# jamie8johnson/cqs

Hardware: AMD Instinct MI355X
Metric: queries/sec @k=20 (brute-force cosine scan + top-k, 768-d fp32) (higher is better)
Workload: dtype f32; 1 GPU; BASELINE configs[1]: 1000000 x 768 fp32 unit vectors, 1 query per step, brute-force cosine top-20; mode=single, rows_per_gpu=1000000, total_rows=1000000, dim=768, k=20, parallelism=single GPU, ranks_seen=1

## Files before the change

cqs_amd/csrc/index_shadow.hip:

```cpp
#include <cstdlib>
#include <cstring>
#include <new>

#include "abi_guard.h"
#include "index_internal.h"
#include "scan_bf16.h"
#include "scan_i8.h"

namespace cqs_idx {

constexpr uint64_t kShadowAutoBytes = 1ull << 30;
constexpr uint64_t kShadowFreeMinBytes = 4ull << 30;
constexpr double kShadowFreeFrac = 0.10;
constexpr uint32_t kStatWords = 10, kStatCounts = 3, kStatI8 = 5, kStatI8Counts = 8;

struct Shadow {
    uint16_t* d_bf16 = nullptr;
    uint64_t cap = 0;
    int8_t* d_i8 = nullptr;
    float* d_i8_scale = nullptr;
    double r8 = 0.0, norm8 = 0.0;
    double r = 0.0;
    double norm = 0.0;
    unsigned long long* d_stats = nullptr;
    uint64_t* d_akeys = nullptr;
    uint32_t* d_acounts = nullptr;
    uint64_t* d_ekeys = nullptr;
    uint32_t* d_cert = nullptr;
    float* d_bq = nullptr;
    uint32_t* h_cert = nullptr;
    uint32_t* h_cert_dev = nullptr;
};

static void shadow_device_counts(cqs_hip_index* x, uint32_t first, uint64_t* certified, uint64_t* fallbacks) {
    unsigned long long c[2];
    if (!x->shadow || !x->shadow->d_stats || quiesce(x) != hipSuccess) return;
    hipError_t e = hipMemcpyAsync(c, x->shadow->d_stats + first, sizeof c, hipMemcpyDeviceToHost, x->stream);
    if (e == hipSuccess) e = hipStreamSynchronize(x->stream);
    if (e != hipSuccess) { (void)hipGetLastError(); return; }
    *certified += c[0];
    *fallbacks += c[1];
}

static void i8_free(Shadow* s) {
    hipFree(s->d_i8); hipFree(s->d_i8_scale);
    s->d_i8 = nullptr; s->d_i8_scale = nullptr;
}

void shadow_free(cqs_hip_index* x) {
    Shadow* s = x->shadow;
    if (!s) return;
    uint64_t c = 0, f = 0;
    shadow_device_counts(x, kStatCounts, &c, &f);
    x->stat_certified.fetch_add(c, std::memory_order_relaxed);
    x->stat_fallbacks.fetch_add(f, std::memory_order_relaxed);
    c = f = 0;
    shadow_device_counts(x, kStatI8Counts, &c, &f);
    x->stat_i8_certified.fetch_add(c, std::memory_order_relaxed);
    x->stat_i8_fallbacks.fetch_add(f, std::memory_order_relaxed);
    i8_free(s);
    hipFree(s->d_bf16); hipFree(s->d_stats); hipFree(s->d_akeys); hipFree(s->d_acounts); hipFree(s->d_ekeys);
    hipFree(s->d_cert); hipFree(s->d_bq); hipHostFree(s->h_cert);
    delete s;
    x->shadow = nullptr;
}

static int32_t shadow_convert(cqs_hip_index* x, uint64_t row0, bool* outlier) {
    Shadow* s = x->shadow;
    HIP_TRY(x, hipMemsetAsync(s->d_stats + 2, 0, sizeof(unsigned long long), x->stream));
    HIP_TRY(x, cqs::launch_shadow_build(x->d_rows, s->d_bf16, row0, x->n - row0, x->dim, cqs::shadow_gamma(x->dim),
                                        s->d_stats, x->stream));
    unsigned long long st[3];
    HIP_TRY(x, hipMemcpyAsync(st, s->d_stats, sizeof st, hipMemcpyDeviceToHost, x->stream));
    HIP_TRY(x, hipStreamSynchronize(x->stream));
    double r, m;
    memcpy(&r, &st[0], sizeof r);
    memcpy(&m, &st[1], sizeof m);
    s->r = r * (1.0 + 0x1p-30);
    s->norm = m * (1.0 + 0x1p-30);
    *outlier = st[2] != 0;
    return CQS_HIP_OK;
}

static int32_t i8_convert(cqs_hip_index* x, uint64_t row0) {
    Shadow* s = x->shadow;
    HIP_TRY(x, cqs::launch_i8_build(x->d_rows, s->d_i8, s->d_i8_scale, row0, x->n - row0, x->dim, cqs::i8_gamma(x->dim),
                                    s->d_stats + kStatI8, x->stream));
    unsigned long long st[2];
    HIP_TRY(x, hipMemcpyAsync(st, s->d_stats + kStatI8, sizeof st, hipMemcpyDeviceToHost, x->stream));
    HIP_TRY(x, hipStreamSynchronize(x->stream));
    double r, m;
    memcpy(&r, &st[0], sizeof r);
    memcpy(&m, &st[1], sizeof m);
    s->r8 = r * (1.0 + 0x1p-30);
    s->norm8 = m * (1.0 + 0x1p-30);
// ... 57 lines not shown
    int32_t rc = shadow_convert(x, n_old, &outlier);
    if (rc == CQS_HIP_OK && s->d_i8 && !outlier) rc = i8_convert(x, n_old);
    if (rc != CQS_HIP_OK) return rc;
    if (outlier) {
        shadow_free(x);
        x->last_error = "extend: a new row has a component of magnitude >= 2^64; bf16 shadow turned off";
    }
    return CQS_HIP_OK;
}

static bool dim_ok(uint32_t dim) { return dim % 8u == 0u && dim <= cqs::kShadowMaxDim; }
static const char* const kDimRule = ": dim must be a multiple of 8 and <= 2048";

static int32_t shadow_enable(cqs_hip_index* x, const char* what) {
    std::string pre(what);
    if (!dim_ok(x->dim)) return fail(x, CQS_HIP_ERR_INVALID, (pre + kDimRule).c_str());
    if (x->shadow) return CQS_HIP_OK;
    auto oom = [&](hipError_t e) { (void)hipGetLastError(); shadow_free(x); return fail(x, CQS_HIP_ERR_NOMEM, (pre + ": allocation").c_str(), e); };
    Shadow* s = x->shadow = new (std::nothrow) Shadow();
    if (!s) return oom(hipErrorOutOfMemory);
    const uint64_t cap = x->cap_rows ? x->cap_rows : 1;
    hipError_t e;
    if ((e = hipMalloc(&s->d_bf16, (size_t)cap * x->dim * sizeof(uint16_t))) != hipSuccess) return oom(e);
    s->cap = cap;
    unsigned long long* stats = nullptr;
    if ((e = hipMalloc(&stats, kStatWords * sizeof(unsigned long long))) != hipSuccess) return oom(e);
    if ((e = hipMemsetAsync(stats, 0, kStatWords * sizeof(unsigned long long), x->stream)) != hipSuccess) { hipFree(stats); return oom(e); }
    s->d_stats = stats;
    if ((e = hipMalloc(&s->d_akeys, (size_t)cqs::kShadowMaxQ * cqs::kMaxK * sizeof(uint64_t))) != hipSuccess) return oom(e);
    if ((e = hipMalloc(&s->d_acounts, (size_t)cqs::kShadowMaxQ * sizeof(uint32_t))) != hipSuccess) return oom(e);
    if ((e = hipMalloc(&s->d_ekeys, (size_t)cqs::kShadowMaxQ * (cqs::kMaxK - 1) * sizeof(uint64_t))) != hipSuccess) return oom(e);
    if ((e = hipMalloc(&s->d_cert, (size_t)cqs::kShadowMaxQ * sizeof(uint32_t))) != hipSuccess) return oom(e);
    if ((e = hipMalloc(&s->d_bq, (size_t)cqs::kShadowMaxQ * sizeof(float))) != hipSuccess) return oom(e);
    if ((e = hipHostMalloc(&s->h_cert, (size_t)cqs::kShadowMaxQ * sizeof(uint32_t), hipHostMallocDefault)) != hipSuccess) return oom(e);
    if (hipHostGetDevicePointer((void**)&s->h_cert_dev, s->h_cert, 0) != hipSuccess) {
        (void)hipGetLastError();
        s->h_cert_dev = nullptr;
    }
    bool outlier = false;
    const int32_t rc = shadow_convert(x, 0, &outlier);
    if (rc != CQS_HIP_OK) { shadow_free(x); return rc; }
    if (outlier) {
        shadow_free(x);
        return fail(x, CQS_HIP_ERR_INVALID, (pre + ": a finite row has a component of magnitude >= 2^64").c_str());
    }
    return CQS_HIP_OK;
}

static bool i8_dim_ok(uint32_t dim) { return cqs::i8_dim_ok(dim); }
static const char* const kI8DimRule = ": dim must be a multiple of 16 and <= 2048";
static int32_t i8_auto(cqs_hip_index* x) {
    Shadow* s = x->shadow;
    if (!s || s->d_i8) return CQS_HIP_OK;
    const char* env = getenv("CQS_HIP_SCAN_I8");
    if (env && env[0] == '0') return CQS_HIP_OK;
    if (!(env && env[0] == '1') && x->n * x->dim * sizeof(float) < kShadowAutoBytes) return CQS_HIP_OK;
    const std::string pre("int8 copy of the shadow not built (the bf16 copy serves every block)");
    if (!i8_dim_ok(x->dim)) { x->last_error = pre + kI8DimRule; return CQS_HIP_OK; }
    size_t free_b = 0, total_b = 0;
    if (hipMemGetInfo(&free_b, &total_b) != hipSuccess) {
        (void)hipGetLastError();
        x->last_error = pre + ": hipMemGetInfo failed";
        return CQS_HIP_OK;
    }
    const uint64_t need = i8_bytes(s->cap, x->dim);
    const uint64_t frac = (uint64_t)(kShadowFreeFrac * (double)total_b);
// ... 25 lines not shown
        (void)hipGetLastError();
        x->last_error = "bf16 shadow not built: hipMemGetInfo failed";
        return CQS_HIP_OK;
    }
    const uint64_t cap = x->cap_rows ? x->cap_rows : 1;
    const uint64_t need = cap * x->dim * sizeof(uint16_t) + (2ull * cqs::kMaxK + 2ull) * cqs::kShadowMaxQ * sizeof(uint64_t);
    const uint64_t frac = (uint64_t)(kShadowFreeFrac * (double)total_b);
    const uint64_t reserve = frac > kShadowFreeMinBytes ? frac : kShadowFreeMinBytes;
    if (free_b < need || free_b - need < reserve) {
        x->last_error = "bf16 shadow not built: the device would keep less than max(4 GiB, 10 %) of its memory free";
        return CQS_HIP_OK;
    }
    int32_t rc = shadow_enable(x, "bf16 shadow not built");
    if (rc == CQS_HIP_OK) rc = i8_auto(x);
    return rc == CQS_HIP_ERR_DEVICE ? rc : CQS_HIP_OK;
}

bool shadow_takes(const cqs_hip_index* x, uint32_t b, uint32_t k, bool gemv_only) {
    return x->shadow && b <= cqs::kShadowMaxQ && (gemv_only || !cqs::use_mfma(b, x->dim)) && cqs::shadow_kprime(k) >= k;
}

bool shadow_uses_i8(const cqs_hip_index* x, uint32_t b, uint32_t k) {
    return x->shadow && x->shadow->d_i8 && b <= cqs::kI8MaxQ && cqs::i8_k_ok(k);
}

int32_t shadow_pass(cqs_hip_index* x, const float* d_q, uint32_t nb, uint32_t k, const uint32_t* d_keep, uint32_t mode,
                    float threshold, uint64_t* out_keys, uint32_t* out_counts, hipStream_t st, const uint32_t** device_gate) {
    const Shadow* s = x->shadow;
    uint32_t* const cert = device_gate || !s->h_cert_dev ? s->d_cert : s->h_cert_dev;
    if (device_gate) *device_gate = cert;
    if (device_gate) HIP_TRY(x, order_after_last(x, st));
    const bool i8 = shadow_uses_i8(x, nb, k);
    const uint32_t kp = i8 ? cqs::i8_kprime(k) : cqs::shadow_kprime(k);
    if (i8) HIP_TRY(x, cqs::launch_i8_bound(d_q, nb, x->dim, s->r8, s->norm8, s->d_bq, st));
    else HIP_TRY(x, cqs::launch_shadow_bound(d_q, nb, x->dim, s->r, s->norm, s->d_bq, st));
    const cqs::ScanArgs a = scan_args(x, d_q, nb, kp + 1u, d_keep, mode, threshold, i8 ? sizeof(int8_t) : sizeof(uint16_t), true, nullptr, nullptr);
    const ShadowRows rows{i8 ? nullptr : s->d_bf16, i8 ? s->d_i8 : nullptr, s->d_i8_scale, s->d_bq};
    const int32_t rc = scan_select(x, a, st, &rows, s->d_akeys, s->d_acounts);
    if (rc == CQS_HIP_OK)
        HIP_TRY(x, cqs::launch_rescore_certify(x->d_rows, x->dim, d_q, nb, k, kp, mode, threshold, (uint32_t)x->row_base,
                                               s->d_bq, s->d_akeys, s->d_acounts, s->d_ekeys, out_keys, out_counts, cert,
                                               device_gate ? s->d_stats + kStatCounts : nullptr,
                                               device_gate && i8 ? s->d_stats + kStatI8Counts : nullptr, st));
    return rc;
}

hipError_t shadow_verdicts(cqs_hip_index* x, uint32_t nb, const uint32_t** h_cert) {
    const Shadow* s = x->shadow;
    *h_cert = s->h_cert;
    return s->h_cert_dev ? hipSuccess : hipMemcpyAsync(s->h_cert, s->d_cert, (size_t)nb * sizeof(uint32_t), hipMemcpyDeviceToHost, x->stream);
}

}

using namespace cqs_idx;

extern "C" {

int32_t cqs_hip_index_set_bf16_scan(cqs_hip_index* x, int32_t enable) CQS_ABI_TRY {
    if (!x || x->sh) return CQS_HIP_ERR_INVALID;
    std::lock_guard<std::mutex> g(x->mu);
    if (x->poisoned.load(std::memory_order_acquire)) return CQS_HIP_ERR_POISONED;
    HIP_TRY(x, hipSetDevice(x->device));
    HIP_TRY(x, quiesce(x));
    if (!enable) { shadow_free(x); return CQS_HIP_OK; }
    if (x->borrow) return fail(x, CQS_HIP_ERR_INVALID, "set_bf16_scan: index borrows its rows (they may change under the bound)");
    const int32_t rc = shadow_enable(x, "set_bf16_scan");
    return rc == CQS_HIP_OK ? i8_auto(x) : rc;
} CQS_ABI_CATCH(x)

void cqs_hip_index_bf16_stats(const cqs_hip_index* x, uint64_t* bytes, uint64_t* certified, uint64_t* fallbacks) CQS_ABI_TRY {
    uint64_t by = 0, c = 0, f = 0;
    if (x && !x->sh) {
        cqs_hip_index* m = const_cast<cqs_hip_index*>(x);
// ... 41 lines not shown
    for (uint32_t i = 0; i < b; ++i) {
        const float* q = queries + (size_t)i * x->dim;
        double s2 = 0.0;
        for (uint32_t d = 0; d < x->dim; ++d) s2 += (double)q[d] * (double)q[d];
        out_host[i] = cqs::shadow_query_bound(s2, s->r, s->norm, x->dim);
    }
    return CQS_HIP_OK;
} CQS_ABI_CATCH(x)

int32_t cqs_hip_debug_shadow_bound_i8(cqs_hip_index* x, const float* queries, uint32_t b, float* out_device, float* out_host) CQS_ABI_TRY {
    if (!x || x->sh || !queries || !out_device || !out_host || b == 0) return CQS_HIP_ERR_INVALID;
    std::lock_guard<std::mutex> g(x->mu);
    const Shadow* s = x->shadow;
    if (!s || !s->d_i8 || b > cqs::kShadowMaxQ) return CQS_HIP_ERR_INVALID;
    HIP_TRY(x, hipSetDevice(x->device));
    HIP_TRY(x, quiesce(x));
    float* d_q = nullptr;
    HIP_TRY(x, hipMalloc(&d_q, (size_t)b * x->dim * sizeof(float)));
    hipError_t e = hipMemcpyAsync(d_q, queries, (size_t)b * x->dim * sizeof(float), hipMemcpyHostToDevice, x->stream);
    if (e == hipSuccess) e = cqs::launch_i8_bound(d_q, b, x->dim, s->r8, s->norm8, s->d_bq, x->stream);
    if (e == hipSuccess) e = hipMemcpyAsync(out_device, s->d_bq, (size_t)b * sizeof(float), hipMemcpyDeviceToHost, x->stream);
    if (e == hipSuccess) e = hipStreamSynchronize(x->stream);
    hipFree(d_q);
    HIP_TRY(x, e);
    for (uint32_t i = 0; i < b; ++i) {
        const float* q = queries + (size_t)i * x->dim;
        double s2 = 0.0;
        for (uint32_t d = 0; d < x->dim; ++d) s2 += (double)q[d] * (double)q[d];
        out_host[i] = cqs::i8_query_bound(s2, s->r8, s->norm8, x->dim);
    }
    return CQS_HIP_OK;
} CQS_ABI_CATCH(x)

int32_t cqs_hip_debug_shadow_stats(cqs_hip_index* x, double* out) CQS_ABI_TRY {
    if (!x || x->sh || !out) return CQS_HIP_ERR_INVALID;
    std::lock_guard<std::mutex> g(x->mu);
    const Shadow* s = x->shadow;
    if (!s) return CQS_HIP_ERR_INVALID;
    out[0] = s->r; out[1] = s->norm;
    out[2] = s->d_i8 ? s->r8 : 0.0; out[3] = s->d_i8 ? s->norm8 : 0.0;
    return CQS_HIP_OK;
} CQS_ABI_CATCH(x)

int32_t cqs_hip_debug_shadow_rows(cqs_hip_index* x, uint32_t copy, uint64_t row0, uint64_t rows, void* out, float* out_scales) CQS_ABI_TRY {
    if (!x || x->sh || !out || (copy != 1u && copy != 2u) || (copy == 2u && !out_scales)) return CQS_HIP_ERR_INVALID;
    std::lock_guard<std::mutex> g(x->mu);
    const Shadow* s = x->shadow;
    if (!s || (copy == 2u && !s->d_i8) || row0 > x->n || rows > x->n - row0) return CQS_HIP_ERR_INVALID;
    if (rows == 0) return CQS_HIP_OK;
    HIP_TRY(x, hipSetDevice(x->device));
    HIP_TRY(x, quiesce(x));
    if (copy == 1u) {
        HIP_TRY(x, hipMemcpyAsync(out, s->d_bf16 + row0 * x->dim, (size_t)rows * x->dim * sizeof(uint16_t), hipMemcpyDeviceToHost, x->stream));
    } else {
        HIP_TRY(x, hipMemcpyAsync(out, s->d_i8 + row0 * x->dim, (size_t)rows * x->dim, hipMemcpyDeviceToHost, x->stream));
        HIP_TRY(x, hipMemcpyAsync(out_scales, s->d_i8_scale + row0, (size_t)rows * sizeof(float), hipMemcpyDeviceToHost, x->stream));
    }
    HIP_TRY(x, hipStreamSynchronize(x->stream));
    return CQS_HIP_OK;
} CQS_ABI_CATCH(x)

int32_t cqs_hip_debug_shadow_scores(cqs_hip_index* x, uint32_t copy, const float* queries, uint32_t b, uint32_t k,
                                    const uint32_t* keep_bitset, uint32_t mode, float threshold, float* out_scores,
                                    float* out_bq) CQS_ABI_TRY {
    if (!x || x->sh || !queries || !out_scores || !out_bq || b == 0 || copy > 2u || mode > CQS_HIP_MODE_PIPELINE) return CQS_HIP_ERR_INVALID;
    if (k == 0 || k > cqs::kMaxK) return CQS_HIP_ERR_INVALID;
// ... 39 lines not shown
```

cqs_amd/csrc/scan_bf16.h:

```cpp
#pragma once
#include <math.h>
#include <stdint.h>

#if defined(__HIPCC__)
#include <hip/hip_runtime.h>
#include "scan_kernels.h"
#define CQS_HD __host__ __device__
#else
#define CQS_HD
#endif

namespace cqs {

constexpr uint32_t kShadowMaxQ = 32;
constexpr uint32_t kShadowMaxDim = 2048;
constexpr uint32_t kShadowKMax = 1024;

inline uint32_t shadow_kprime(uint32_t k) {
    const uint32_t kp = 2u * k + 32u;
    return kp < kShadowKMax - 1u ? kp : kShadowKMax - 1u;
}

CQS_HD inline double shadow_gamma(uint32_t dim) {
    const double du = (double)dim * 0x1p-24;
    return du / (1.0 - du);
}

CQS_HD inline float round_up_f32(double v) {
    float f = (float)v;
    if ((double)f < v) f = nextafterf(f, INFINITY);
    return f;
}

CQS_HD inline float shadow_query_bound(double q_norm2, double r_max, double norm_max, uint32_t dim) {
    const double qn = sqrt(q_norm2) * (1.0 + 0x1p-40);
    if (!(qn * norm_max * (1.0 + shadow_gamma(dim)) < 0x1p100)) return INFINITY;
    return round_up_f32(qn * r_max * (1.0 + 0x1p-40) + (double)dim * 0x1p-140);
}

#if defined(__HIPCC__)
hipError_t launch_shadow_build(const float* rows, uint16_t* shadow, uint64_t row0, uint64_t n_rows, uint32_t dim,
                               double gamma, unsigned long long* stats, hipStream_t st);

hipError_t launch_shadow_bound(const float* q, uint32_t b, uint32_t dim, double r_max, double norm_max, float* bq,
                               hipStream_t st);

hipError_t launch_scan_bf16(const ScanArgs& a, const uint16_t* shadow, const float* bq, hipStream_t st);

hipError_t launch_rescore_certify(const float* rows, uint32_t dim, const float* q, uint32_t b, uint32_t k, uint32_t kprime,
                                  uint32_t mode, float thr, uint32_t row_base, const float* bq, const uint64_t* akeys,
                                  const uint32_t* acounts, uint64_t* ekeys, uint64_t* out_keys, uint32_t* out_counts,
                                  uint32_t* cert, unsigned long long* counters, unsigned long long* counters2, hipStream_t st);
#endif

}
```

cqs_amd/csrc/scan_bf16.hip:

```cpp
#include "scan_bf16.h"
#include "launch_util.h"
#include "rank_sort.h"
#include "scan_device.h"

namespace cqs {

static_assert(kShadowKMax == kMaxK, "shadow k' policy and the select agree on max k");

typedef float f4 __attribute__((ext_vector_type(4)));
typedef float f2 __attribute__((ext_vector_type(2)));
typedef unsigned u4 __attribute__((ext_vector_type(4)));
typedef __bf16 bf2 __attribute__((ext_vector_type(2)));

__device__ __forceinline__ float bf_lo(uint32_t w) { return __uint_as_float(w << 16); }
__device__ __forceinline__ float bf_hi(uint32_t w) { return __uint_as_float(w & 0xFFFF0000u); }
__device__ __forceinline__ float key_score(uint64_t key) {
    const uint32_t ok = (uint32_t)(key >> 32);
    return __uint_as_float((ok & 0x80000000u) ? (ok ^ 0x80000000u) : ~ok);
}

__global__ __launch_bounds__(256) void shadow_build_kernel(const float* __restrict__ rows, uint16_t* __restrict__ shadow,
                                                           uint64_t row0, uint64_t n_rows, uint32_t dim, double gamma,
                                                           unsigned long long* __restrict__ stats) {
    const int lane = threadIdx.x & 63;
    const uint64_t waves = (uint64_t)gridDim.x * (blockDim.x >> 6);
    for (uint64_t r = (uint64_t)blockIdx.x * (blockDim.x >> 6) + (threadIdx.x >> 6); r < n_rows; r += waves) {
        const float* xp = rows + (row0 + r) * dim;
        uint16_t* op = shadow + (row0 + r) * dim;
        double d2 = 0.0, n2 = 0.0, t2 = 0.0;
        bool fin = true, big = false;
        for (uint32_t i = (uint32_t)lane * 2u; i < dim; i += 128u) {
            const f2 v = *(const f2*)(xp + i);
            const bf2 h = __builtin_convertvector(v, bf2);
// ... 7 lines not shown
            n2 += (double)v.x * (double)v.x + (double)v.y * (double)v.y;
            t2 += (double)t0 * (double)t0 + (double)t1 * (double)t1;
        }
#pragma unroll
        for (int m = 32; m >= 1; m >>= 1) {
            d2 += __shfl_xor(d2, m, 64);
            n2 += __shfl_xor(n2, m, 64);
            t2 += __shfl_xor(t2, m, 64);
        }
        const bool all_fin = __ballot(!fin) == 0ull;
        const bool any_big = __ballot(big) != 0ull;
        if (lane == 0 && all_fin) {
            const double nx = sqrt(n2), nt = sqrt(t2);
            const double rb = sqrt(d2) + gamma * (nx + nt);
            atomicMax(&stats[0], (unsigned long long)__double_as_longlong(rb));
            atomicMax(&stats[1], (unsigned long long)__double_as_longlong(nx > nt ? nx : nt));
            if (any_big) atomicMax(&stats[2], 1ull);
        }
    }
}

hipError_t launch_shadow_build(const float* rows, uint16_t* shadow, uint64_t row0, uint64_t n_rows, uint32_t dim,
                               double gamma, unsigned long long* stats, hipStream_t st) {
    if (n_rows == 0) return hipSuccess;
    const uint64_t blocks = (n_rows + 3u) / 4u;
    hipLaunchKernelGGL(shadow_build_kernel, dim3((uint32_t)(blocks < 8192u ? blocks : 8192u)), dim3(256), 0, st, rows,
                       shadow, row0, n_rows, dim, gamma, stats);
    return hipGetLastError();
}

__global__ __launch_bounds__(64) void shadow_bound_kernel(const float* __restrict__ q, uint32_t dim, double r_max,
                                                          double norm_max, float* __restrict__ bq) {
    const uint32_t lane = threadIdx.x;
    const float* qp = q + (size_t)blockIdx.x * dim;
    double s2 = 0.0;
    for (uint32_t d = lane; d < dim; d += 64u) s2 += (double)qp[d] * (double)qp[d];
#pragma unroll
    for (int m = 32; m >= 1; m >>= 1) s2 += __shfl_xor(s2, m, 64);
    if (lane == 0) bq[blockIdx.x] = shadow_query_bound(s2, r_max, norm_max, dim);
}

hipError_t launch_shadow_bound(const float* q, uint32_t b, uint32_t dim, double r_max, double norm_max, float* bq,
                               hipStream_t st) {
    if (b == 0) return hipSuccess;
    if (b > kShadowMaxQ) return hipErrorInvalidValue;
    hipLaunchKernelGGL(shadow_bound_kernel, dim3(b), dim3(64), 0, st, q, dim, r_max, norm_max, bq);
    return hipGetLastError();
}

struct Bf16ScanParams {
    const uint16_t* rows;
    uint32_t n, n_pad, dim;
    const float* q;
    float* scores;
    const uint32_t* keep;
    uint32_t mode;
    float thr;
    uint32_t nq;
    uint32_t* work;
    TaskTiers tiers;
    uint32_t n_tasks;
    float* gmax;
    uint64_t* gaux;
    const float* bq;
};

template <int NCH, int BQ, int RI, bool NT, bool FULL>
__global__ __launch_bounds__(256) void scan_bf16_kernel(const Bf16ScanParams p) {
    constexpr int NV = RI * BQ;
    constexpr int LPV = 64 / NV;
    const int lane = threadIdx.x & 63;
    const uint32_t n = p.n, dim = p.dim;
// ... 175 lines not shown
    uint32_t done = 0, slot = 0;
    while (done < a.b) {
        const uint32_t left = a.b - done;
        hipError_t e;
        uint32_t g;
        if constexpr (NCH <= 2) {
            if (left >= 5) { g = left < 8u ? left : 8u; e = launch_bf16<NCH, 8, 2>(a, shadow, bq, done, g, slot, st); }
            else if (left >= 4) { g = 4; e = launch_bf16<NCH, 4, 4>(a, shadow, bq, done, g, slot, st); }
            else if (left >= 2) { g = 2; e = launch_bf16<NCH, 2, 8>(a, shadow, bq, done, g, slot, st); }
            else { g = 1; e = launch_bf16<NCH, 1, 16>(a, shadow, bq, done, g, slot, st); }
        } else {
            if (left >= 2) { g = 2; e = launch_bf16<NCH, 2, 4>(a, shadow, bq, done, g, slot, st); }
            else { g = 1; e = launch_bf16<NCH, 1, 8>(a, shadow, bq, done, g, slot, st); }
        }
        if (e != hipSuccess) return e;
        done += g;
        slot = (slot + 1u) % kWorkWords;
    }
    return hipSuccess;
}

hipError_t launch_scan_bf16(const ScanArgs& a, const uint16_t* shadow, const float* bq, hipStream_t st) {
    if (a.b == 0 || a.n == 0) return hipSuccess;
    if (a.b > kShadowMaxQ || a.dim % 8u != 0u || a.dim > kShadowMaxDim) return hipErrorInvalidValue;
    switch ((a.dim + 511u) / 512u) {
        case 1: return launch_bf16_groups<1>(a, shadow, bq, st);
        case 2: return launch_bf16_groups<2>(a, shadow, bq, st);
        case 3: return launch_bf16_groups<3>(a, shadow, bq, st);
        case 4: return launch_bf16_groups<4>(a, shadow, bq, st);
        default: return hipErrorInvalidValue;
    }
}

struct RescoreParams {
    const float* rows;
    const float* q;
    uint32_t dim, kprime, mode, row_base;
    float thr;
    const uint64_t* akeys;
    const uint32_t* acounts;
    uint64_t* ekeys;
};

template <int NCH>
__global__ __launch_bounds__(256) void rescore_kernel(const RescoreParams p) {
    const int lane = threadIdx.x & 63;
    const uint32_t qi = blockIdx.y;
    const uint32_t i = blockIdx.x * 4u + (threadIdx.x >> 6);
    const uint32_t ac = p.acounts[qi];
    const uint32_t cnt = ac < p.kprime ? ac : p.kprime;
    if (i >= cnt) return;
    const uint64_t key = p.akeys[(size_t)qi * (p.kprime + 1u) + i];
    const uint32_t grow = 0xFFFFFFFFu - (uint32_t)key;
    const uint32_t dim = p.dim;
    const float* rp = p.rows + (size_t)(grow - p.row_base) * dim;
    const float* qp = p.q + (size_t)qi * dim;
    f4 x[NCH], qv[NCH];
#pragma unroll
    for (int c = 0; c < NCH; ++c) {
        const uint32_t idx = (uint32_t)c * 256u + (uint32_t)lane * 4u;
        const bool in = idx < dim;
        const uint32_t off = in ? idx : dim - 4u;
        x[c] = *(const f4*)(rp + off);
        const f4 v = *(const f4*)(qp + off);
        qv[c] = in ? v : (f4)(0.f);
    }
    f2 acc2 = (f2)(0.f);
#pragma unroll
    for (int c = 0; c < NCH; ++c) {
        const f2 xlo = __builtin_shufflevector(x[c], x[c], 0, 1);
        const f2 xhi = __builtin_shufflevector(x[c], x[c], 2, 3);
        acc2 = __builtin_elementwise_fma(xlo, __builtin_shufflevector(qv[c], qv[c], 0, 1), acc2);
        acc2 = __builtin_elementwise_fma(xhi, __builtin_shufflevector(qv[c], qv[c], 2, 3), acc2);
    }
    float s = acc2.x + acc2.y;
#pragma unroll
    for (int m = 32; m >= 1; m >>= 1) s += __shfl_xor(s, m, 64);
    bool keep = __builtin_fabsf(s) <= 3.4028234664e38f;
    if (keep && p.mode == 1u) {
        s = s < 0.f ? 0.f : (s > 1.f ? 1.f : s);
        keep = s >= p.thr;
    }
    if (lane == 0) p.ekeys[(size_t)qi * p.kprime + i] = keep ? pack_key(okey(s), grow) : 0ull;
}

struct CertifyParams {
    const uint64_t* ekeys;
    const uint64_t* akeys;
    const uint32_t* acounts;
    uint32_t k, kprime, mode;
    uint64_t* out_keys;
    uint32_t* out_counts;
    uint32_t* cert;
    const float* bq;
    unsigned long long* counters;
    unsigned long long* counters2;
};

__global__ __launch_bounds__(1024) void certify_kernel(const CertifyParams p) {
    __shared__ uint64_t s_keys[kShadowKMax];
    __shared__ uint64_t s_sorted[kShadowKMax];
    __shared__ __attribute__((aligned(16))) uint32_t s_ok[kShadowKMax + 4];
    __shared__ uint32_t s_cnt, s_flag;
    const uint32_t qi = blockIdx.x;
    const uint32_t ac = p.acounts[qi];
    const uint32_t nc = ac < p.kprime ? ac : p.kprime;
    if (threadIdx.x == 0) s_cnt = 0u;
    __syncthreads();
    if (threadIdx.x < nc) {
        const uint64_t key = p.ekeys[(size_t)qi * p.kprime + threadIdx.x];
        if (key != 0ull) s_keys[atomicAdd(&s_cnt, 1u)] = key;
    }
    __syncthreads();
    const uint32_t m = s_cnt;
    rank_sort_keys(s_keys, m, s_sorted, s_ok, &s_flag);
    const uint32_t k = p.k;
    const uint32_t outc = m < k ? m : k;
    for (uint32_t i = threadIdx.x; i < k; i += 1024u) p.out_keys[(size_t)qi * k + i] = (i < outc) ? s_sorted[i] : 0ull;
    if (threadIdx.x == 0) {
        p.out_counts[qi] = outc;
        const float bq = p.bq[qi];
        bool ok = false;
        if (__builtin_fabsf(bq) <= 3.4028234664e38f) {
            if (ac <= p.kprime) ok = true;
            else if (m >= k) {
                float t = key_score(p.akeys[(size_t)qi * (p.kprime + 1u) + p.kprime]) + bq;
                if (p.mode == 1u) t = t < 0.f ? 0.f : (t > 1.f ? 1.f : t);
                ok = t < key_score(s_sorted[k - 1u]);
            }
        }
        p.cert[qi] = ok ? 1u : 0u;
        if (p.counters) atomicAdd(&p.counters[ok ? 0 : 1], 1ull);
        if (p.counters2) atomicAdd(&p.counters2[ok ? 0 : 1], 1ull);
    }
}

hipError_t launch_rescore_certify(const float* rows, uint32_t dim, const float* q, uint32_t b, uint32_t k, uint32_t kprime,
                                  uint32_t mode, float thr, uint32_t row_base, const float* bq, const uint64_t* akeys,
                                  const uint32_t* acounts, uint64_t* ekeys, uint64_t* out_keys, uint32_t* out_counts,
                                  uint32_t* cert, unsigned long long* counters, unsigned long long* counters2, hipStream_t st) {
    if (b == 0) return hipSuccess;
    if (b > kShadowMaxQ || k == 0 || kprime < k || kprime >= kShadowKMax || dim % 8u != 0u || dim > kShadowMaxDim)
        return hipErrorInvalidValue;
    RescoreParams rp{rows, q, dim, kprime, mode, row_base, thr, akeys, acounts, ekeys};
    const dim3 grid((kprime + 3u) / 4u, b), block(256);
    switch ((dim + 255u) / 256u) {
        case 1: hipLaunchKernelGGL(rescore_kernel<1>, grid, block, 0, st, rp); break;
        case 2: hipLaunchKernelGGL(rescore_kernel<2>, grid, block, 0, st, rp); break;
        case 3: hipLaunchKernelGGL(rescore_kernel<3>, grid, block, 0, st, rp); break;
        case 4: hipLaunchKernelGGL(rescore_kernel<4>, grid, block, 0, st, rp); break;
        case 5: hipLaunchKernelGGL(rescore_kernel<5>, grid, block, 0, st, rp); break;
        case 6: hipLaunchKernelGGL(rescore_kernel<6>, grid, block, 0, st, rp); break;
        case 7: hipLaunchKernelGGL(rescore_kernel<7>, grid, block, 0, st, rp); break;
        case 8: hipLaunchKernelGGL(rescore_kernel<8>, grid, block, 0, st, rp); break;
        default: return hipErrorInvalidValue;
    }
    hipError_t e = hipGetLastError();
    if (e != hipSuccess) return e;
    CertifyParams cp{ekeys, akeys, acounts, k, kprime, mode, out_keys, out_counts, cert, bq, counters, counters2};
    hipLaunchKernelGGL(certify_kernel, dim3(b), dim3(1024), 0, st, cp);
    return hipGetLastError();
}

}
```

cqs_amd/csrc/scan_i8.h:

```cpp
#pragma once
#include "scan_bf16.h"

namespace cqs {

constexpr uint32_t kI8MaxQ = 4;

inline uint32_t i8_kprime(uint32_t k) { return 10u * k + 150u; }
inline bool i8_k_ok(uint32_t k) { return i8_kprime(k) <= kShadowKMax - 1u; }

inline bool i8_dim_ok(uint32_t dim) { return dim % 16u == 0u && dim <= kShadowMaxDim; }

CQS_HD inline double i8_gamma(uint32_t dim) { return shadow_gamma(dim + 2u); }

CQS_HD inline float i8_query_bound(double q_norm2, double r_max, double norm_max, uint32_t dim) {
    const double qn = sqrt(q_norm2) * (1.0 + 0x1p-40);
    if (!(qn * norm_max * (1.0 + i8_gamma(dim)) < 0x1p100)) return INFINITY;
    if (!(qn * 128.0 * sqrt((double)dim) < 0x1p100)) return INFINITY;
    return round_up_f32(qn * r_max * (1.0 + 0x1p-40) + (double)dim * 0x1p-140 * (1.0 + norm_max));
}

#if defined(__HIPCC__)
hipError_t launch_i8_build(const float* rows, int8_t* codes, float* scales, uint64_t row0, uint64_t n_rows, uint32_t dim,
                           double gamma, unsigned long long* stats, hipStream_t st);

hipError_t launch_i8_bound(const float* q, uint32_t b, uint32_t dim, double r_max, double norm_max, float* bq, hipStream_t st);

hipError_t launch_scan_i8(const ScanArgs& a, const int8_t* codes, const float* scales, const float* bq, hipStream_t st);
#endif

}
```

cqs_amd/csrc/scan_i8.hip:

```cpp
#include "scan_i8.h"
#include "launch_util.h"
#include "scan_device.h"

namespace cqs {

typedef float f4 __attribute__((ext_vector_type(4)));
typedef float f2 __attribute__((ext_vector_type(2)));
typedef unsigned u4 __attribute__((ext_vector_type(4)));

template <int I>
__device__ __forceinline__ float code_f32(uint32_t w) { return (float)(int)(int8_t)(w >> (8 * I)); }

constexpr int kI8BuildVecs = (int)(kShadowMaxDim / 256u);

__global__ __launch_bounds__(256) void i8_build_kernel(const float* __restrict__ rows, int8_t* __restrict__ codes,
                                                       float* __restrict__ scales, uint64_t row0, uint64_t n_rows,
                                                       uint32_t dim, double gamma, unsigned long long* __restrict__ stats) {
    const uint32_t lane = threadIdx.x & 63u;
    const uint64_t waves = (uint64_t)gridDim.x * (blockDim.x >> 6);
    for (uint64_t r = (uint64_t)blockIdx.x * (blockDim.x >> 6) + (threadIdx.x >> 6); r < n_rows; r += waves) {
        const float* xp = rows + (row0 + r) * dim;
        int8_t* op = codes + (row0 + r) * dim;
        f4 v[kI8BuildVecs];
        float m = 0.f;
// ... 32 lines not shown
            *(uint32_t*)(op + i) = w;
        }
#pragma unroll
        for (int s = 32; s >= 1; s >>= 1) {
            d2 += __shfl_xor(d2, s, 64);
            n2 += __shfl_xor(n2, s, 64);
            t2 += __shfl_xor(t2, s, 64);
        }
        if (lane == 0u) {
            scales[row0 + r] = scale;
            if (all_fin) {
                const double nx = sqrt(n2), nt = sqrt(t2);
                atomicMax(&stats[0], (unsigned long long)__double_as_longlong(sqrt(d2) + gamma * (nx + nt)));
                atomicMax(&stats[1], (unsigned long long)__double_as_longlong(nx > nt ? nx : nt));
                if (m >= 0x1p64f) atomicMax(&stats[2], 1ull);
            }
        }
    }
}

hipError_t launch_i8_build(const float* rows, int8_t* codes, float* scales, uint64_t row0, uint64_t n_rows, uint32_t dim,
                           double gamma, unsigned long long* stats, hipStream_t st) {
    if (n_rows == 0) return hipSuccess;
    if (!i8_dim_ok(dim)) return hipErrorInvalidValue;
    const uint64_t blocks = (n_rows + 3u) / 4u;
    hipLaunchKernelGGL(i8_build_kernel, dim3((uint32_t)(blocks < 8192u ? blocks : 8192u)), dim3(256), 0, st, rows, codes,
                       scales, row0, n_rows, dim, gamma, stats);
    return hipGetLastError();
}

__global__ __launch_bounds__(64) void i8_bound_kernel(const float* __restrict__ q, uint32_t dim, double r_max,
                                                      double norm_max, float* __restrict__ bq) {
    const uint32_t lane = threadIdx.x;
    const float* qp = q + (size_t)blockIdx.x * dim;
    double s2 = 0.0;
    for (uint32_t d = lane; d < dim; d += 64u) s2 += (double)qp[d] * (double)qp[d];
#pragma unroll
    for (int m = 32; m >= 1; m >>= 1) s2 += __shfl_xor(s2, m, 64);
    if (lane == 0) bq[blockIdx.x] = i8_query_bound(s2, r_max, norm_max, dim);
}

hipError_t launch_i8_bound(const float* q, uint32_t b, uint32_t dim, double r_max, double norm_max, float* bq, hipStream_t st) {
    if (b == 0) return hipSuccess;
    if (b > kShadowMaxQ) return hipErrorInvalidValue;
    hipLaunchKernelGGL(i8_bound_kernel, dim3(b), dim3(64), 0, st, q, dim, r_max, norm_max, bq);
    return hipGetLastError();
}

struct I8ScanParams {
    const int8_t* rows;
    const float* scales;
    uint32_t n, n_pad, dim;
    const float* q;
    float* scores;
    const uint32_t* keep;
    uint32_t mode;
    float thr;
    uint32_t nq;
    TaskTiers tiers;
    uint32_t n_tasks;
    float* gmax;
    uint64_t* gaux;
    const float* bq;
};

template <int NCH, int BQ, int RI, bool NT, bool FULL>
__global__ __launch_bounds__(256) void scan_i8_kernel(const I8ScanParams p) {
    constexpr int NV = RI * BQ;
    constexpr int LPV = 64 / NV;
    const int lane = threadIdx.x & 63;
    const uint32_t n = p.n, dim = p.dim;

// ... 186 lines not shown
```

Baseline: 6123 queries/s.

## Fuse rescore, certify and query-bound kernels into one ticketed tail kernel

Merges the separate rescore and certify kernels into a single launch where every block rescores candidates and the last block to arrive, found through a per-query atomic ticket counter, performs the sort and certification. Outside pipeline mode, the query-bound computation also moves into a spare wave of that tail kernel instead of running as its own launch before the scan. The aim is to cut per-query launch overhead, which matters at batch size 1. The cost is a last-block-done pattern that relies on atomics and explicit waitcnt ordering, plus a persistent ticket buffer that has to be reset correctly.

```diff
diff --git a/cqs_amd/csrc/index_shadow.hip b/cqs_amd/csrc/index_shadow.hip
--- a/cqs_amd/csrc/index_shadow.hip
+++ b/cqs_amd/csrc/index_shadow.hip
@@ -28,6 +28,7 @@
     uint64_t* d_ekeys = nullptr;
     uint32_t* d_cert = nullptr;
     float* d_bq = nullptr;
+    uint32_t* d_tickets = nullptr;
     uint32_t* h_cert = nullptr;
     uint32_t* h_cert_dev = nullptr;
 };
@@ -60,7 +61,7 @@
     x->stat_i8_fallbacks.fetch_add(f, std::memory_order_relaxed);
     i8_free(s);
     hipFree(s->d_bf16); hipFree(s->d_stats); hipFree(s->d_akeys); hipFree(s->d_acounts); hipFree(s->d_ekeys);
-    hipFree(s->d_cert); hipFree(s->d_bq); hipHostFree(s->h_cert);
+    hipFree(s->d_cert); hipFree(s->d_bq); hipFree(s->d_tickets); hipHostFree(s->h_cert);
     delete s;
     x->shadow = nullptr;
 }
@@ -184,6 +185,8 @@
     if ((e = hipMalloc(&s->d_ekeys, (size_t)cqs::kShadowMaxQ * (cqs::kMaxK - 1) * sizeof(uint64_t))) != hipSuccess) return oom(e);
     if ((e = hipMalloc(&s->d_cert, (size_t)cqs::kShadowMaxQ * sizeof(uint32_t))) != hipSuccess) return oom(e);
     if ((e = hipMalloc(&s->d_bq, (size_t)cqs::kShadowMaxQ * sizeof(float))) != hipSuccess) return oom(e);
+    if ((e = hipMalloc(&s->d_tickets, (size_t)cqs::kShadowMaxQ * sizeof(uint32_t))) != hipSuccess) return oom(e);
+    if ((e = hipMemsetAsync(s->d_tickets, 0, (size_t)cqs::kShadowMaxQ * sizeof(uint32_t), x->stream)) != hipSuccess) return oom(e);
     if ((e = hipHostMalloc(&s->h_cert, (size_t)cqs::kShadowMaxQ * sizeof(uint32_t), hipHostMallocDefault)) != hipSuccess) return oom(e);
     if (hipHostGetDevicePointer((void**)&s->h_cert_dev, s->h_cert, 0) != hipSuccess) {
         (void)hipGetLastError();
@@ -275,14 +278,19 @@
     if (device_gate) HIP_TRY(x, order_after_last(x, st));
     const bool i8 = shadow_uses_i8(x, nb, k);
     const uint32_t kp = i8 ? cqs::i8_kprime(k) : cqs::shadow_kprime(k);
-    if (i8) HIP_TRY(x, cqs::launch_i8_bound(d_q, nb, x->dim, s->r8, s->norm8, s->d_bq, st));
-    else HIP_TRY(x, cqs::launch_shadow_bound(d_q, nb, x->dim, s->r, s->norm, s->d_bq, st));
+    const double r_max = i8 ? s->r8 : s->r, norm_max = i8 ? s->norm8 : s->norm;
+    const bool bound_first = mode == CQS_HIP_MODE_PIPELINE;
+    if (bound_first) {
+        if (i8) HIP_TRY(x, cqs::launch_i8_bound(d_q, nb, x->dim, r_max, norm_max, s->d_bq, st));
+        else HIP_TRY(x, cqs::launch_shadow_bound(d_q, nb, x->dim, r_max, norm_max, s->d_bq, st));
+    }
     const cqs::ScanArgs a = scan_args(x, d_q, nb, kp + 1u, d_keep, mode, threshold, i8 ? sizeof(int8_t) : sizeof(uint16_t), true, nullptr, nullptr);
     const ShadowRows rows{i8 ? nullptr : s->d_bf16, i8 ? s->d_i8 : nullptr, s->d_i8_scale, s->d_bq};
     const int32_t rc = scan_select(x, a, st, &rows, s->d_akeys, s->d_acounts);
     if (rc == CQS_HIP_OK)
         HIP_TRY(x, cqs::launch_rescore_certify(x->d_rows, x->dim, d_q, nb, k, kp, mode, threshold, (uint32_t)x->row_base,
-                                               s->d_bq, s->d_akeys, s->d_acounts, s->d_ekeys, out_keys, out_counts, cert,
+                                               bound_first ? 0u : (i8 ? 2u : 1u), r_max, norm_max, s->d_bq, s->d_tickets,
+                                               s->d_akeys, s->d_acounts, s->d_ekeys, out_keys, out_counts, cert,
                                                device_gate ? s->d_stats + kStatCounts : nullptr,
                                                device_gate && i8 ? s->d_stats + kStatI8Counts : nullptr, st));
     return rc;
@@ -390,6 +398,18 @@
     return CQS_HIP_OK;
 } CQS_ABI_CATCH(x)
 
+int32_t cqs_hip_debug_shadow_bq(cqs_hip_index* x, uint32_t b, float* out) CQS_ABI_TRY {
+    if (!x || x->sh || !out || b == 0) return CQS_HIP_ERR_INVALID;
+    std::lock_guard<std::mutex> g(x->mu);
+    const Shadow* s = x->shadow;
+    if (!s || b > cqs::kShadowMaxQ) return CQS_HIP_ERR_INVALID;
+    HIP_TRY(x, hipSetDevice(x->device));
+    HIP_TRY(x, quiesce(x));
+    HIP_TRY(x, hipMemcpyAsync(out, s->d_bq, (size_t)b * sizeof(float), hipMemcpyDeviceToHost, x->stream));
+    HIP_TRY(x, hipStreamSynchronize(x->stream));
+    return CQS_HIP_OK;
+} CQS_ABI_CATCH(x)
+
 int32_t cqs_hip_debug_shadow_stats(cqs_hip_index* x, double* out) CQS_ABI_TRY {
     if (!x || x->sh || !out) return CQS_HIP_ERR_INVALID;
     std::lock_guard<std::mutex> g(x->mu);
diff --git a/cqs_amd/csrc/scan_bf16.h b/cqs_amd/csrc/scan_bf16.h
--- a/cqs_amd/csrc/scan_bf16.h
+++ b/cqs_amd/csrc/scan_bf16.h
@@ -39,6 +39,17 @@
 }
 
 #if defined(__HIPCC__)
+__device__ __forceinline__ double wave_q_norm2(const float* qp, uint32_t dim, uint32_t lane) {
+    double s2 = 0.0;
+    for (uint32_t d = lane; d < dim; d += 64u) s2 += (double)qp[d] * (double)qp[d];
+#pragma unroll
+    for (int m = 32; m >= 1; m >>= 1) s2 += __shfl_xor(s2, m, 64);
+    return s2;
+}
+__device__ __forceinline__ float wave_shadow_bound(const float* qp, uint32_t dim, double r_max, double norm_max, uint32_t lane) {
+    return shadow_query_bound(wave_q_norm2(qp, dim, lane), r_max, norm_max, dim);
+}
+
 hipError_t launch_shadow_build(const float* rows, uint16_t* shadow, uint64_t row0, uint64_t n_rows, uint32_t dim,
                                double gamma, unsigned long long* stats, hipStream_t st);
 
@@ -48,9 +59,10 @@
 hipError_t launch_scan_bf16(const ScanArgs& a, const uint16_t* shadow, const float* bq, hipStream_t st);
 
 hipError_t launch_rescore_certify(const float* rows, uint32_t dim, const float* q, uint32_t b, uint32_t k, uint32_t kprime,
-                                  uint32_t mode, float thr, uint32_t row_base, const float* bq, const uint64_t* akeys,
-                                  const uint32_t* acounts, uint64_t* ekeys, uint64_t* out_keys, uint32_t* out_counts,
-                                  uint32_t* cert, unsigned long long* counters, unsigned long long* counters2, hipStream_t st);
+                                  uint32_t mode, float thr, uint32_t row_base, uint32_t bound, double r_max, double norm_max,
+                                  float* bq, uint32_t* tickets, const uint64_t* akeys, const uint32_t* acounts,
+                                  uint64_t* ekeys, uint64_t* out_keys, uint32_t* out_counts, uint32_t* cert,
+                                  unsigned long long* counters, unsigned long long* counters2, hipStream_t st);
 #endif
 
 }
diff --git a/cqs_amd/csrc/scan_bf16.hip b/cqs_amd/csrc/scan_bf16.hip
--- a/cqs_amd/csrc/scan_bf16.hip
+++ b/cqs_amd/csrc/scan_bf16.hip
@@ -1,4 +1,5 @@
 #include "scan_bf16.h"
+#include "scan_i8.h"
 #include "launch_util.h"
 #include "rank_sort.h"
 #include "scan_device.h"
@@ -72,12 +73,8 @@
 __global__ __launch_bounds__(64) void shadow_bound_kernel(const float* __restrict__ q, uint32_t dim, double r_max,
                                                           double norm_max, float* __restrict__ bq) {
     const uint32_t lane = threadIdx.x;
-    const float* qp = q + (size_t)blockIdx.x * dim;
-    double s2 = 0.0;
-    for (uint32_t d = lane; d < dim; d += 64u) s2 += (double)qp[d] * (double)qp[d];
-#pragma unroll
-    for (int m = 32; m >= 1; m >>= 1) s2 += __shfl_xor(s2, m, 64);
-    if (lane == 0) bq[blockIdx.x] = shadow_query_bound(s2, r_max, norm_max, dim);
+    const float v = wave_shadow_bound(q + (size_t)blockIdx.x * dim, dim, r_max, norm_max, lane);
+    if (lane == 0) bq[blockIdx.x] = v;
 }
 
 hipError_t launch_shadow_bound(const float* q, uint32_t b, uint32_t dim, double r_max, double norm_max, float* bq,
@@ -319,83 +316,96 @@
     }
 }
 
-struct RescoreParams {
+struct TailParams {
     const float* rows;
     const float* q;
-    uint32_t dim, kprime, mode, row_base;
+    uint32_t dim, k, kprime, mode, row_base;
     float thr;
     const uint64_t* akeys;
     const uint32_t* acounts;
     uint64_t* ekeys;
-};
-
-template <int NCH>
-__global__ __launch_bounds__(256) void rescore_kernel(const RescoreParams p) {
-    const int lane = threadIdx.x & 63;
-    const uint32_t qi = blockIdx.y;
-    const uint32_t i = blockIdx.x * 4u + (threadIdx.x >> 6);
-    const uint32_t ac = p.acounts[qi];
-    const uint32_t cnt = ac < p.kprime ? ac : p.kprime;
-    if (i >= cnt) return;
-    const uint64_t key = p.akeys[(size_t)qi * (p.kprime + 1u) + i];
-    const uint32_t grow = 0xFFFFFFFFu - (uint32_t)key;
-    const uint32_t dim = p.dim;
-    const float* rp = p.rows + (size_t)(grow - p.row_base) * dim;
-    const float* qp = p.q + (size_t)qi * dim;
-    f4 x[NCH], qv[NCH];
-#pragma unroll
-    for (int c = 0; c < NCH; ++c) {
-        const uint32_t idx = (uint32_t)c * 256u + (uint32_t)lane * 4u;
-        const bool in = idx < dim;
-        const uint32_t off = in ? idx : dim - 4u;
-        x[c] = *(const f4*)(rp + off);
-        const f4 v = *(const f4*)(qp + off);
-        qv[c] = in ? v : (f4)(0.f);
-    }
-    f2 acc2 = (f2)(0.f);
-#pragma unroll
-    for (int c = 0; c < NCH; ++c) {
-        const f2 xlo = __builtin_shufflevector(x[c], x[c], 0, 1);
-        const f2 xhi = __builtin_shufflevector(x[c], x[c], 2, 3);
-        acc2 = __builtin_elementwise_fma(xlo, __builtin_shufflevector(qv[c], qv[c], 0, 1), acc2);
-        acc2 = __builtin_elementwise_fma(xhi, __builtin_shufflevector(qv[c], qv[c], 2, 3), acc2);
-    }
-    float s = acc2.x + acc2.y;
-#pragma unroll
-    for (int m = 32; m >= 1; m >>= 1) s += __shfl_xor(s, m, 64);
-    bool keep = __builtin_fabsf(s) <= 3.4028234664e38f;
-    if (keep && p.mode == 1u) {
-        s = s < 0.f ? 0.f : (s > 1.f ? 1.f : s);
-        keep = s >= p.thr;
-    }
-    if (lane == 0) p.ekeys[(size_t)qi * p.kprime + i] = keep ? pack_key(okey(s), grow) : 0ull;
-}
-
-struct CertifyParams {
-    const uint64_t* ekeys;
-    const uint64_t* akeys;
-    const uint32_t* acounts;
-    uint32_t k, kprime, mode;
+    float* bq;
+    uint32_t* tickets;
+    uint32_t bound;
+    double r_max, norm_max;
     uint64_t* out_keys;
     uint32_t* out_counts;
     uint32_t* cert;
-    const float* bq;
     unsigned long long* counters;
     unsigned long long* counters2;
 };
 
-__global__ __launch_bounds__(1024) void certify_kernel(const CertifyParams p) {
+constexpr uint32_t kTailWaves = 16;
+
+template <int NCH>
+__global__ __launch_bounds__(1024) void rescore_certify_kernel(const TailParams p) {
     __shared__ uint64_t s_keys[kShadowKMax];
     __shared__ uint64_t s_sorted[kShadowKMax];
     __shared__ __attribute__((aligned(16))) uint32_t s_ok[kShadowKMax + 4];
-    __shared__ uint32_t s_cnt, s_flag;
-    const uint32_t qi = blockIdx.x;
+    __shared__ uint32_t s_cnt, s_flag, s_last;
+    const uint32_t lane = threadIdx.x & 63u;
+    const uint32_t qi = blockIdx.y;
+    const uint32_t slot = (uint32_t)__builtin_amdgcn_readfirstlane((int)(blockIdx.x * kTailWaves + (threadIdx.x >> 6)));
     const uint32_t ac = p.acounts[qi];
     const uint32_t nc = ac < p.kprime ? ac : p.kprime;
+    const uint32_t dim = p.dim;
+    const float* qp = p.q + (size_t)qi * dim;
     if (threadIdx.x == 0) s_cnt = 0u;
+    if (slot == 0u) {
+        if (p.bound != 0u) {
+            const float v = p.bound == 2u ? wave_i8_bound(qp, dim, p.r_max, p.norm_max, lane)
+                                          : wave_shadow_bound(qp, dim, p.r_max, p.norm_max, lane);
+            if (lane == 0u)
+                __hip_atomic_store((uint32_t*)p.bq + qi, __float_as_uint(v), __ATOMIC_RELAXED, __HIP_MEMORY_SCOPE_AGENT);
+        }
+    } else if (slot - 1u < nc) {
+        const uint32_t i = slot - 1u;
+        const uint64_t key = p.akeys[(size_t)qi * (p.kprime + 1u) + i];
+        const uint32_t grow = 0xFFFFFFFFu - (uint32_t)key;
+        const float* rp = p.rows + (size_t)(grow - p.row_base) * dim;
+        f4 x[NCH], qv[NCH];
+#pragma unroll
+        for (int c = 0; c < NCH; ++c) {
+            const uint32_t idx = (uint32_t)c * 256u + lane * 4u;
+            const bool in = idx < dim;
+            const uint32_t off = in ? idx : dim - 4u;
+            x[c] = *(const f4*)(rp + off);
+            const f4 v = *(const f4*)(qp + off);
+            qv[c] = in ? v : (f4)(0.f);
+        }
+        f2 acc2 = (f2)(0.f);
+#pragma unroll
+        for (int c = 0; c < NCH; ++c) {
+            const f2 xlo = __builtin_shufflevector(x[c], x[c], 0, 1);
+            const f2 xhi = __builtin_shufflevector(x[c], x[c], 2, 3);
+            acc2 = __builtin_elementwise_fma(xlo, __builtin_shufflevector(qv[c], qv[c], 0, 1), acc2);
+            acc2 = __builtin_elementwise_fma(xhi, __builtin_shufflevector(qv[c], qv[c], 2, 3), acc2);
+        }
+        float s = acc2.x + acc2.y;
+#pragma unroll
+        for (int m = 32; m >= 1; m >>= 1) s += __shfl_xor(s, m, 64);
+        bool keep = __builtin_fabsf(s) <= 3.4028234664e38f;
+        if (keep && p.mode == 1u) {
+            s = s < 0.f ? 0.f : (s > 1.f ? 1.f : s);
+            keep = s >= p.thr;
+        }
+        if (lane == 0u)
+            __hip_atomic_store(p.ekeys + (size_t)qi * p.kprime + i, keep ? pack_key(okey(s), grow) : 0ull, __ATOMIC_RELAXED,
+                               __HIP_MEMORY_SCOPE_AGENT);
+    }
+    asm volatile("s_waitcnt vmcnt(0)" ::: "memory");
     __syncthreads();
+    if (threadIdx.x == 0) {
+        const uint32_t t = __hip_atomic_fetch_add(p.tickets + qi, 1u, __ATOMIC_RELAXED, __HIP_MEMORY_SCOPE_AGENT);
+        const bool last = t == gridDim.x - 1u;
+        if (last) __hip_atomic_store(p.tickets + qi, 0u, __ATOMIC_RELAXED, __HIP_MEMORY_SCOPE_AGENT);
+        s_last = last ? 1u : 0u;
+    }
+    __syncthreads();
+    if (s_last == 0u) return;
+
     if (threadIdx.x < nc) {
-        const uint64_t key = p.ekeys[(size_t)qi * p.kprime + threadIdx.x];
+        const uint64_t key = __hip_atomic_load(p.ekeys + (size_t)qi * p.kprime + threadIdx.x, __ATOMIC_RELAXED, __HIP_MEMORY_SCOPE_AGENT);
         if (key != 0ull) s_keys[atomicAdd(&s_cnt, 1u)] = key;
     }
     __syncthreads();
@@ -406,7 +416,7 @@
     for (uint32_t i = threadIdx.x; i < k; i += 1024u) p.out_keys[(size_t)qi * k + i] = (i < outc) ? s_sorted[i] : 0ull;
     if (threadIdx.x == 0) {
         p.out_counts[qi] = outc;
-        const float bq = p.bq[qi];
+        const float bq = __uint_as_float(__hip_atomic_load((uint32_t*)p.bq + qi, __ATOMIC_RELAXED, __HIP_MEMORY_SCOPE_AGENT));
         bool ok = false;
         if (__builtin_fabsf(bq) <= 3.4028234664e38f) {
             if (ac <= p.kprime) ok = true;
@@ -423,29 +433,27 @@
 }
 
 hipError_t launch_rescore_certify(const float* rows, uint32_t dim, const float* q, uint32_t b, uint32_t k, uint32_t kprime,
-                                  uint32_t mode, float thr, uint32_t row_base, const float* bq, const uint64_t* akeys,
-                                  const uint32_t* acounts, uint64_t* ekeys, uint64_t* out_keys, uint32_t* out_counts,
-                                  uint32_t* cert, unsigned long long* counters, unsigned long long* counters2, hipStream_t st) {
+                                  uint32_t mode, float thr, uint32_t row_base, uint32_t bound, double r_max, double norm_max,
+                                  float* bq, uint32_t* tickets, const uint64_t* akeys, const uint32_t* acounts,
+                                  uint64_t* ekeys, uint64_t* out_keys, uint32_t* out_counts, uint32_t* cert,
+                                  unsigned long long* counters, unsigned long long* counters2, hipStream_t st) {
     if (b == 0) return hipSuccess;
-    if (b > kShadowMaxQ || k == 0 || kprime < k || kprime >= kShadowKMax || dim % 8u != 0u || dim > kShadowMaxDim)
+    if (b > kShadowMaxQ || k == 0 || kprime < k || kprime >= kShadowKMax || dim % 8u != 0u || dim > kShadowMaxDim || bound > 2u)
         return hipErrorInvalidValue;
-    RescoreParams rp{rows, q, dim, kprime, mode, row_base, thr, akeys, acounts, ekeys};
-    const dim3 grid((kprime + 3u) / 4u, b), block(256);
+    const TailParams tp{rows, q, dim, k, kprime, mode, row_base, thr, akeys, acounts, ekeys, bq, tickets, bound, r_max, norm_max,
+                        out_keys, out_counts, cert, counters, counters2};
+    const dim3 grid((kprime + 1u + kTailWaves - 1u) / kTailWaves, b), block(64u * kTailWaves);
     switch ((dim + 255u) / 256u) {
-        case 1: hipLaunchKernelGGL(rescore_kernel<1>, grid, block, 0, st, rp); break;
-        case 2: hipLaunchKernelGGL(rescore_kernel<2>, grid, block, 0, st, rp); break;
-        case 3: hipLaunchKernelGGL(rescore_kernel<3>, grid, block, 0, st, rp); break;
-        case 4: hipLaunchKernelGGL(rescore_kernel<4>, grid, block, 0, st, rp); break;
-        case 5: hipLaunchKernelGGL(rescore_kernel<5>, grid, block, 0, st, rp); break;
-        case 6: hipLaunchKernelGGL(rescore_kernel<6>, grid, block, 0, st, rp); break;
-        case 7: hipLaunchKernelGGL(rescore_kernel<7>, grid, block, 0, st, rp); break;
-        case 8: hipLaunchKernelGGL(rescore_kernel<8>, grid, block, 0, st, rp); break;
+        case 1: hipLaunchKernelGGL(rescore_certify_kernel<1>, grid, block, 0, st, tp); break;
+        case 2: hipLaunchKernelGGL(rescore_certify_kernel<2>, grid, block, 0, st, tp); break;
+        case 3: hipLaunchKernelGGL(rescore_certify_kernel<3>, grid, block, 0, st, tp); break;
+        case 4: hipLaunchKernelGGL(rescore_certify_kernel<4>, grid, block, 0, st, tp); break;
+        case 5: hipLaunchKernelGGL(rescore_certify_kernel<5>, grid, block, 0, st, tp); break;
+        case 6: hipLaunchKernelGGL(rescore_certify_kernel<6>, grid, block, 0, st, tp); break;
+        case 7: hipLaunchKernelGGL(rescore_certify_kernel<7>, grid, block, 0, st, tp); break;
+        case 8: hipLaunchKernelGGL(rescore_certify_kernel<8>, grid, block, 0, st, tp); break;
         default: return hipErrorInvalidValue;
     }
-    hipError_t e = hipGetLastError();
-    if (e != hipSuccess) return e;
-    CertifyParams cp{ekeys, akeys, acounts, k, kprime, mode, out_keys, out_counts, cert, bq, counters, counters2};
-    hipLaunchKernelGGL(certify_kernel, dim3(b), dim3(1024), 0, st, cp);
     return hipGetLastError();
 }
 
diff --git a/cqs_amd/csrc/scan_i8.h b/cqs_amd/csrc/scan_i8.h
--- a/cqs_amd/csrc/scan_i8.h
+++ b/cqs_amd/csrc/scan_i8.h
@@ -20,6 +20,10 @@
 }
 
 #if defined(__HIPCC__)
+__device__ __forceinline__ float wave_i8_bound(const float* qp, uint32_t dim, double r_max, double norm_max, uint32_t lane) {
+    return i8_query_bound(wave_q_norm2(qp, dim, lane), r_max, norm_max, dim);
+}
+
 hipError_t launch_i8_build(const float* rows, int8_t* codes, float* scales, uint64_t row0, uint64_t n_rows, uint32_t dim,
                            double gamma, unsigned long long* stats, hipStream_t st);
 
diff --git a/cqs_amd/csrc/scan_i8.hip b/cqs_amd/csrc/scan_i8.hip
--- a/cqs_amd/csrc/scan_i8.hip
+++ b/cqs_amd/csrc/scan_i8.hip
@@ -88,12 +88,8 @@
 __global__ __launch_bounds__(64) void i8_bound_kernel(const float* __restrict__ q, uint32_t dim, double r_max,
                                                       double norm_max, float* __restrict__ bq) {
     const uint32_t lane = threadIdx.x;
-    const float* qp = q + (size_t)blockIdx.x * dim;
-    double s2 = 0.0;
-    for (uint32_t d = lane; d < dim; d += 64u) s2 += (double)qp[d] * (double)qp[d];
-#pragma unroll
-    for (int m = 32; m >= 1; m >>= 1) s2 += __shfl_xor(s2, m, 64);
-    if (lane == 0) bq[blockIdx.x] = i8_query_bound(s2, r_max, norm_max, dim);
+    const float v = wave_i8_bound(q + (size_t)blockIdx.x * dim, dim, r_max, norm_max, lane);
+    if (lane == 0) bq[blockIdx.x] = v;
 }
 
 hipError_t launch_i8_bound(const float* q, uint32_t b, uint32_t dim, double r_max, double norm_max, float* bq, hipStream_t st) {
```

Measured after the change: 6369 queries/s (median of 6 runs). +4.0%, better.
